# kiva12138/MIMRL

Measured on AMD Instinct MI355X. Metric: two-stage train iters/sec, higher is better.
Workload: dtype bf16

## Files before the change

mimrl_amd/csrc/cube_fused.h:

```cpp
#pragma once
#include "common.h"
#include "model_ops.h"

namespace mimrl {

struct CubeFusedArgs {
  const float* x;
  const float *l_w1, *l_b1, *l_w2, *l_b2, *l_wr, *l_g, *l_be;
  KMixW kw;
  const float *d_w1, *d_b1, *d_w2, *d_b2, *d_wr, *d_g, *d_be;
  float *l_u, *l_h, *l_y, *l_z, *l_mean, *l_rstd;
  float* k_z;
  float *d_u, *d_h, *d_y, *d_mean, *d_rstd;
  float* d_z;
  int B, il, hl, ol, K, act, save;
  int dbg_phase;
};

bool cube_fused_supported(int il, int hl, int ol, int ik, int hk, int ok, int id, int hd, int od, bool ln_first,
                          bool res_project, bool bias, const float* dropout_mlp);
int cube_block_fwd_fused(hipStream_t s, const CubeFusedArgs& a);

#ifdef MIMRL_PHASE_PROBE
int cube_fwd_read_phases(long long* out);
#endif

}
```

mimrl_amd/csrc/cube_fused.hip:

```cpp
#include "cube_fused.h"

#include "kmix_device.h"

#include <type_traits>

namespace mimrl {

namespace {

constexpr int D = 128;
constexpr int ILD = 72;
constexpr int IMG = 64 * ILD;
constexpr int CTL = 68, CTD = 132;

typedef _Float16 bf;

#ifdef MIMRL_PHASE_PROBE
__device__ long long g_cube_phase[128];
#define CPHASE(i) do { if (blockIdx.x == 0 && threadIdx.x == 0) g_cube_phase[(SAVE ? 64 : 0) + (NMT - 1) * 16 + (i)] = (long long)wall_clock64(); } while (0)
#else
#define CPHASE(i) do { } while (0)
#endif

__device__ __forceinline__ void mma64(f32x16& acc, const bf* A, const bf* B, int wm, int wn, int lane) {
#pragma unroll
  for (int s = 0; s < 4; ++s) {
    const f16x8 a = *reinterpret_cast<const f16x8*>(A + (wm * 32 + (lane & 31)) * ILD + s * 16 + 8 * (lane >> 5));
    const f16x8 b = *reinterpret_cast<const f16x8*>(B + (wn * 32 + (lane & 31)) * ILD + s * 16 + 8 * (lane >> 5));
    acc = __builtin_amdgcn_mfma_f32_32x32x16_f16(a, b, acc, 0, 0, 0);
  }
}
__device__ __forceinline__ int acc_row(int r, int wm, int lane) { return wm * 32 + (r & 3) + 8 * (r >> 2) + 4 * (lane >> 5); }

struct WReq { float v[16]; };
// ... 60 lines not shown
  c.prm = c.ksw + 256 * 4;
  const int l_end = c.prm + 4 * 64 * 4;
  c.bw = 0;
  c.dprm = c.bw + 2 * G * IMG * 2;
  int after = c.dprm + 2 * D * 4;
  if (after < xm_bytes) after = xm_bytes;
  c.az = (after + 15) & ~15;
  c.ah = c.az + nmt * 2 * IMG * 2;
  const int ah_bytes = nmt * 2 * IMG * 2, ctd_bytes = 64 * CTD * 4;
  c.ctd = c.ah;
  const int d_end = c.ah + (ah_bytes > ctd_bytes ? ah_bytes : ctd_bytes);
  c.total = l_end > d_end ? l_end : d_end;
  return c;
}

template <bool SAVE, int NMT, int G>
__global__ __launch_bounds__(256 * G) void cube_fwd_fused_kernel(CubeFusedArgs a) {
  extern __shared__ __attribute__((aligned(16))) char smem[];
  constexpr int NT = 256 * G;
  const int tid = threadIdx.x, grp = tid >> 8, t = tid & 255, lane = t & 63, wave = t >> 6, wm = wave >> 1, wn = wave & 1;
  const int b = blockIdx.x;
  const int K = a.K, C = K * D, XP = C + 8, il = a.il, hl = a.hl, ol = a.ol;
  const Carve cv = carve(K, NMT, G);
  bf* Xm = reinterpret_cast<bf*>(smem + cv.xm);
  bf* Aw = reinterpret_cast<bf*>(smem + cv.aw);
  bf* Bx = reinterpret_cast<bf*>(smem + cv.bx) + grp * IMG;
  bf* Bh = reinterpret_cast<bf*>(smem + cv.bh) + grp * IMG;
  float* CtL = reinterpret_cast<float*>(smem + cv.ctl) + grp * 64 * CTL;
  float* red = reinterpret_cast<float*>(smem + cv.red) + grp * 2 * 4 * 64;
  float* ksw = reinterpret_cast<float*>(smem + cv.ksw);
  float* prm = reinterpret_cast<float*>(smem + cv.prm);

  CPHASE(0);
  {
    const bool g0 = G == 1 || grp == 0;
    const WReq w0 = stage_weight_request(g0 ? a.l_w1 : a.l_w2, g0 ? il : hl, 0, 0, g0 ? hl : ol, g0 ? il : hl, t);
    const WReq w1 = stage_weight_request(a.l_wr, il, 0, 0, ol, il, t);
    WReq w2;
    if (G == 1) w2 = stage_weight_request(a.l_w2, hl, 0, 0, ol, hl, t);
    float pr[4] = {0.f, 0.f, 0.f, 0.f};
    if (tid < 64) {
      pr[0] = (tid < hl && a.l_b1) ? a.l_b1[tid] : 0.f;
      pr[1] = (tid < ol && a.l_b2) ? a.l_b2[tid] : 0.f;
      pr[2] = tid < ol ? a.l_g[tid] : 0.f;
      pr[3] = tid < ol ? a.l_be[tid] : 0.f;
    }
    CPHASE(13);
    const float* xb = a.x + (long)b * il * C;
    const int nq = C / 4, total = 64 * nq;
    constexpr int NQ = SAVE ? 6 : 12;
    for (int i0 = tid; i0 < total; i0 += NT * NQ) {
      float4 q[NQ];
#pragma unroll
      for (int j = 0; j < NQ; ++j) {
        const int i = i0 + NT * j;
        const int ic = i < total ? i : total - 1;
        const int l = ic / nq, c4 = (ic - l * nq) * 4;
        q[j] = *reinterpret_cast<const float4*>(xb + (long)(l < il ? l : il - 1) * C + c4);
      }
#pragma unroll
      for (int j = 0; j < NQ; ++j) {
        const int i = i0 + NT * j;
        if (!(i < total && i / nq < il)) q[j] = make_float4(0.f, 0.f, 0.f, 0.f);
      }
#pragma unroll
      for (int j = 0; j < NQ; ++j) {
        const int i = i0 + NT * j;
        if (i < total) {
          const int l = i / nq, c4 = (i - l * nq) * 4;
          f16x4 p; p[0] = to_f16_sat(q[j].x); p[1] = to_f16_sat(q[j].y); p[2] = to_f16_sat(q[j].z); p[3] = to_f16_sat(q[j].w);
          *reinterpret_cast<f16x4*>(Xm + l * XP + c4) = p;
        }
      }
    }
    CPHASE(14);
    if (tid < 64) { prm[0 * 64 + tid] = pr[0]; prm[1 * 64 + tid] = pr[1]; prm[2 * 64 + tid] = pr[2]; prm[3 * 64 + tid] = pr[3]; }
    stage_weight_commit(g0 ? Aw + 0 * IMG : Aw + 1 * IMG, w0, 0, 0, g0 ? hl : ol, g0 ? il : hl, t);
    if (g0) stage_weight_commit(Aw + 2 * IMG, w1, 0, 0, ol, il, t);
    if (G == 1) stage_weight_commit(Aw + 1 * IMG, w2, 0, 0, ol, hl, t);
  }
  __syncthreads();
  CPHASE(1);
  if (a.dbg_phase == 1) return;

  for (int nb = 0; nb < C; nb += 64 * G) {
    const int n0 = nb + 64 * grp;
    const bool on = n0 < C;
    if (on) {
// ... 123 lines not shown
        }
      }
      });
    };
    if (K == 3) phase_k(std::integral_constant<int, 3>{});
    else if (K == 1) phase_k(std::integral_constant<int, 1>{});
    else if (K == 2) phase_k(std::integral_constant<int, 2>{});
    else phase_k(std::integral_constant<int, 4>{});
  }
  __syncthreads();

  CPHASE(3);
  if (a.dbg_phase == 3) return;
  const int R = ol * K;
  float* CtD = reinterpret_cast<float*>(smem + cv.ctd);
  float* dgam = reinterpret_cast<float*>(smem + cv.dprm);
  float* dbet = dgam + D;
  bf* Az = reinterpret_cast<bf*>(smem + cv.az);
  bf* Ah = reinterpret_cast<bf*>(smem + cv.ah);
  for (int c = tid; c < NMT * 64 * 16; c += NT) {
    const int r = c >> 4, ch = c & 15;
    f16x8 v;
#pragma unroll
    for (int j = 0; j < 8; ++j) v[j] = to_f16(0.f);
    if (r < R) {
      const int l = r / K, kk = r - l * K;
      v = *reinterpret_cast<const f16x8*>(Xm + l * XP + kk * D + ch * 8);
    }
    *reinterpret_cast<f16x8*>(Az + ((r >> 6) * 2 + (ch >> 3)) * IMG + (r & 63) * ILD + (ch & 7) * 8) = v;
  }
  __syncthreads();
// ... 61 lines not shown
  CPHASE(5);
  if (a.dbg_phase == 4) return;
#pragma unroll
  for (int i = NI1; i < 3 * NI1; ++i) {
    const int which = i >= 2 * NI1, q = (i % NI1) >> 1, kh = i & 1;
    commit_weight128(Bw2[i & 1], wnext, t);
    if (i + 1 < 3 * NI1) wnext = wload(i + 1);
    __syncthreads();
    const bf* Asrc = which == 0 ? Ah : Az;
#pragma unroll
    for (int mt = 0; mt < NMT; ++mt) mma64(acc[mt][q], Asrc + (mt * 2 + kh) * IMG, Bw2[i & 1], wm, wn, lane);
  }
  __syncthreads();
  CPHASE(6);
  if (a.dbg_phase == 5) return;
#pragma unroll
  for (int mt = 0; mt < NMT; ++mt) {
#pragma unroll
    for (int q = 0; q < NTW; ++q) {
      const int n = wn * 32 + (lane & 31), col = (nt0 + q) * 64 + n;
      const float b2 = b2v[q];
#pragma unroll
      for (int r = 0; r < 16; ++r) CtD[acc_row(r, wm, lane) * CTD + col] = acc[mt][q][r] + b2;
    }
    __syncthreads();
    {
      constexpr int TPR = 4 * G, CW = 32 / G;
      const int m = tid / TPR, part = tid % TPR, row = mt * 64 + m;
      float yv[CW];
      float s0 = 0.f;
// ... 8 lines not shown
      float v0 = 0.f;
#pragma unroll
      for (int j = 0; j < CW; ++j) { const float c = yv[j] - mu; v0 += c * c; }
      v0 = group_sum<TPR>(v0);
      const float rs = rsqrtf(v0 * (1.f / D) + LN_EPS);
      if (row < R) {
        const long o = ((long)b * R + row) * D + part * CW;
#pragma unroll
        for (int j = 0; j < CW / 4; ++j) {
          const int c = part * CW + 4 * j;
          float4 z;
          z.x = (yv[4 * j] - mu) * rs * dgam[c] + dbet[c];
          z.y = (yv[4 * j + 1] - mu) * rs * dgam[c + 1] + dbet[c + 1];
          z.z = (yv[4 * j + 2] - mu) * rs * dgam[c + 2] + dbet[c + 2];
          z.w = (yv[4 * j + 3] - mu) * rs * dgam[c + 3] + dbet[c + 3];
          *reinterpret_cast<float4*>(a.d_z + o + 4 * j) = z;
          if (SAVE) *reinterpret_cast<float4*>(a.d_y + o + 4 * j) = make_float4(yv[4 * j], yv[4 * j + 1], yv[4 * j + 2], yv[4 * j + 3]);
        }
        if (SAVE && part == 0) { a.d_mean[(long)b * R + row] = mu; a.d_rstd[(long)b * R + row] = rs; }
      }
    }
    __syncthreads();
  }
  CPHASE(7);
}

}

#ifdef MIMRL_PHASE_PROBE
int cube_fwd_read_phases(long long* out) { return hipMemcpyFromSymbol(out, HIP_SYMBOL(g_cube_phase), sizeof(long long) * 128) == hipSuccess ? 0 : 1; }
#endif

bool cube_fused_supported(int il, int hl, int ol, int ik, int hk, int ok, int id, int hd, int od, bool ln_first,
                          bool res_project, bool bias, const float* dropout_mlp) {
  (void)bias;
  if (ln_first || !res_project) return false;
  if (dropout_mlp[0] > 0.f || dropout_mlp[1] > 0.f || dropout_mlp[2] > 0.f) return false;
  if (id != D || hd != D || od != D) return false;
  if (il > 64 || hl > 64 || ol > 64 || il < 1 || hl < 1 || ol < 1) return false;
  if (ik != hk || ik != ok || ik < 1 || ik > 4) return false;
  if (ol * ok > 192) return false;
  return true;
}

int cube_block_fwd_fused(hipStream_t s, const CubeFusedArgs& a) {
// ... 10 lines not shown
    HIPX(hipFuncSetAttribute(reinterpret_cast<const void*>(kern), hipFuncAttributeMaxDynamicSharedMemorySize, cv.total)); \
    hipLaunchKernelGGL(kern, dim3(a.B), dim3(256 * GG), cv.total, s, a);                                           \
  } while (0)
#define LAUNCH_NMT(SAVE, GG)                                                                                       \
  do {                                                                                                             \
    if (nmt == 1) LAUNCH_FUSED(SAVE, 1, GG); else if (nmt == 2) LAUNCH_FUSED(SAVE, 2, GG); else LAUNCH_FUSED(SAVE, 3, GG); \
  } while (0)
  if (a.save) { if (G == 1) LAUNCH_NMT(true, 1); else LAUNCH_NMT(true, 2); }
  else { if (G == 1) LAUNCH_NMT(false, 1); else LAUNCH_NMT(false, 2); }
#undef LAUNCH_NMT
#undef LAUNCH_FUSED
  LAUNCH_CHECK();
  return MIMRL_OK;
}

}
```

mimrl_amd/csrc/engine.h:

```cpp
#pragma once
#include <cstdio>
#include <cstdlib>
#include <cstring>
#include <algorithm>
#include <vector>
#include <dlfcn.h>

#include "cube_fused.h"
#include "mlp_fused.h"
#include "concat_fused.h"
#include "cube_bwd_fused.h"
#include "cube_long.h"
#include "estimator_ops.h"
#include "gemm.h"
#include "gru.h"
#include "gru_wgrad.h"
#include "concat_dw.h"
#include "lstm.h"
#include "layout.h"
#include "comm.h"
#include "model_ops.h"

namespace mimrl {

// ... 198 lines not shown
  float *dfeat = nullptr, *dtout = nullptr, *dta[3], *dtin = nullptr, *dca[3], *dP = nullptr, *dQ = nullptr;
  float *dcc[3], *dcin = nullptr;
  static constexpr int NGBUF = 24;
  float* gbuf[NGBUF];
  size_t gbuf_floats = 0;
  float *dtx = nullptr, *ds[2], *dg[2][2][2], *hprev[2][2][2], *dh0[2];

  static constexpr int NSIDE = 6;
  hipStream_t side[NSIDE] = {nullptr, nullptr, nullptr, nullptr, nullptr, nullptr};
  std::vector<hipEvent_t> ev_pool;
  size_t ev_next = 0;
  bool multi_stream = true;
  bool fused_cube_bwd = true;
  bool fused_mlp = true;
  bool fused_cube = true;
  int fwd_f16 = 1;
  int next_event(hipEvent_t* e) {
    if (ev_next == ev_pool.size()) {
      hipEvent_t n;
      HIPX(hipEventCreateWithFlags(&n, hipEventDisableTiming));
      ev_pool.push_back(n);
    }
    *e = ev_pool[ev_next++];
    return MIMRL_OK;
  }
  int G_group(hipStream_t st, const GemmDesc* ds, int n) {
    if (!prof_on) return gemm_group(st, ds, n, bf16);
    for (int i = 0; i < n; ++i) MX(G_on(st, ds[i]));
    return MIMRL_OK;
  }
// ... 143 lines not shown
  int G_(const GemmDesc& d) { return G_on(stream, d); }
  static constexpr bool fp32_site(int) { return false; }
  struct PrecGuard {
    mimrl_handle* h; bool saved;
    PrecGuard(mimrl_handle* h_, bool force_fp32) : h(h_), saved(h_->bf16) { if (force_fp32) h->bf16 = false; }
    ~PrecGuard() { h->bf16 = saved; }
  };
  struct Deferred { int kind; int side; GemmDesc g; const float* src; long n0, n1, n2, n3; float* dst;
                    const float *p1 = nullptr, *p2 = nullptr, *p3 = nullptr; float* dst2 = nullptr; KMixW kw = KMixW();
                    const float *p4 = nullptr, *p5 = nullptr; float *dst3 = nullptr, *dst4 = nullptr; };
  std::vector<Deferred> deferred;
  int flush_deferred(int only_side = 0);
  int wg_helper = -1;
  int dbg_delay(hipStream_t st, int tag);
  int model_forward(bool train, bool save, int knn_stage = 0, int part = 0);
  int cube_forward(bool train, bool save);
  int cube_backward(int cur_in, int* cur_out);
  int wt_images(hipStream_t st, bool bwd_bf16, bool launch, bool* d_fused);
  int model_backward();
  int encoders_backward(float* dcube);
  int gru_layer_backward(int l);
  struct StreamGuard {
    mimrl_handle* h; hipStream_t saved;
    StreamGuard(mimrl_handle* h_, hipStream_t st) : h(h_), saved(h_->stream) { h->stream = st; }
    ~StreamGuard() { h->stream = saved; }
  };
  int knn_launch(int stage, hipStream_t st);
  bool pipe_primed = false; int fwd_parity = 0, pipe_set = 0;
  int pipe_forward_body(bool other_inputs);
  int run_stage1_pipe_prime();
  int run_stage1_pipe(bool next_valid);
// ... 26 lines not shown
```

mimrl_amd/csrc/engine_abi.hip:

```cpp
#include "engine.h"

extern "C" {

const char* mimrl_last_error(void) { return mimrl::last_error_slot().c_str(); }
#ifdef MIMRL_PHASE_PROBE
int mimrl_dbg_cube_phases(long long* out) { return mimrl::cube_fwd_read_phases(out); }
int mimrl_dbg_cube_bwd_phases(long long* out) { return mimrl::cube_bwd_read_phases(out); }
int mimrl_dbg_kmix_phases(long long* out) { return mimrl::kmix_bwd_read_phases(out); }
int mimrl_dbg_nce_phases(long long* out) { return mimrl::nce_read_phases(out); }
int mimrl_dbg_model_ops_phases(long long* out) { return mimrl::model_ops_read_phases(out); }
int mimrl_dbg_gru_bwd_phases(long long* out) { return mimrl::gru_bwd_read_phases(out); }
int mimrl_dbg_concat_bwd_phases(long long* out) { return mimrl::concat_bwd_read_phases(out); }
#endif
int mimrl_abi_version(void) { return MIMRL_ABI_VERSION; }

int mimrl_device_check(void) {
  int n = 0;
  if (hipGetDeviceCount(&n) != hipSuccess || n <= 0) return set_error(MIMRL_ERR_NODEVICE, "no HIP device visible");
  int dev = 0;
  if (hipGetDevice(&dev) != hipSuccess) return set_error(MIMRL_ERR_NODEVICE, "hipGetDevice failed");
  hipDeviceProp_t p;
  if (hipGetDeviceProperties(&p, dev) != hipSuccess) return set_error(MIMRL_ERR_NODEVICE, "hipGetDeviceProperties failed");
  if (std::strncmp(p.gcnArchName, "gfx950", 6) != 0)
    return set_error(MIMRL_ERR_NODEVICE, "device %d is %s; this library is built for gfx950 (MI355X) only", dev, p.gcnArchName);
// ... 18 lines not shown
  MX(mimrl_device_check());
  if (knob_on("MIMRL_KNOBS")) knobs_print(stderr);
  mimrl_handle* h = new (std::nothrow) mimrl_handle();
  if (!h) return set_error(MIMRL_ERR_STATE, "out of host memory");
  h->cfg = *cfg;
  if (h->cfg.beta1 == 0.f) h->cfg.beta1 = 0.9f;
  if (h->cfg.beta2 == 0.f) h->cfg.beta2 = 0.999f;
  if (h->cfg.adam_eps == 0.f) h->cfg.adam_eps = 1e-8f;
  h->stream = h->user_stream = reinterpret_cast<hipStream_t>(hip_stream);
  h->multi_stream = knob("MIMRL_SINGLE_STREAM") == nullptr;
#ifdef MIMRL_DET
  h->multi_stream = false;
  MX(det_init());
#endif
  h->fused_cube = knob("MIMRL_NO_FUSED_CUBE") == nullptr;
  h->fused_mlp = knob("MIMRL_NO_FUSED_MLP") == nullptr;
  h->knn_pre = true;
  h->fold_unpack_on = knob("MIMRL_NO_FOLD_UNPACK") == nullptr;
  h->h16_on = knob("MIMRL_NO_H16") == nullptr;
  h->xin_on = knob("MIMRL_NO_XIN") == nullptr;
  h->fused_cube_bwd = knob("MIMRL_NO_FUSED_CUBE_BWD") == nullptr;
  h->laxis_bwd_long_on = !(knob("MIMRL_LAXIS_BWD_LONG") && atoi(knob("MIMRL_LAXIS_BWD_LONG")) == 0);
  h->laxis_long_on = !(knob("MIMRL_LAXIS_LONG") && atoi(knob("MIMRL_LAXIS_LONG")) == 0);
  h->rec16_on = !(knob("MIMRL_REC16") && atoi(knob("MIMRL_REC16")) == 0);
  h->dwih_h16_on = !(knob("MIMRL_DWIH_H16") && atoi(knob("MIMRL_DWIH_H16")) == 0);
  h->adam_frag_on = !(knob("MIMRL_ADAM_FRAG") && atoi(knob("MIMRL_ADAM_FRAG")) == 0);
  h->fused_concat = knob("MIMRL_NO_FUSED_CONCAT") == nullptr;
  h->fwd_f16 = knob("MIMRL_FWD_BF16") == nullptr;
  h->l0_packed = knob("MIMRL_L0_PACK") ? atoi(knob("MIMRL_L0_PACK")) != 0 : true;
  h->dg_bf16 = cfg->encoder == MIMRL_ENCODER_GRU && (cfg->precision & MIMRL_PREC_BF16_GRU_BWD) && (cfg->precision & MIMRL_PREC_BF16_GEMM_BWD) &&
// ... 687 lines not shown
```

mimrl_amd/csrc/engine_forward.hip:

```cpp
#include "engine.h"

int mimrl_handle::encoders_forward(bool save, int knn_stage) {
  if (cfg.encoder == MIMRL_ENCODER_CONV) return conv_forward(knn_stage);
  if (cfg.encoder == MIMRL_ENCODER_LSTM) return lstm_encoders_forward(save, knn_stage);
  const int B = cfg.batch, T = cfg.seq_len;
  const long BT_ = (long)B * T;
  const float* xin[2] = {bufs.audio, bufs.video};
  const int dmod[2] = {cfg.d_a, cfg.d_v};
  if (!ev_lens) MX(seq_lengths2(S(4), xin[0], dmod[0], lens[0], xin[1], dmod[1], lens[1], B, T));
  const bool use_h16 = h16_on && l0_packed && bf16 && fwd_f16 && (prec & MIMRL_PREC_BF16_GRU_FWD) && !fp32_site(4) && !fp32_site(2) && h0h[0] && w1h;
  if (save) { h16_live = use_h16; hp16_live = false; }
  for (int l = 0; l < 2; ++l) {
    GruFwdArgs a;
    a.B = B; a.T = T; a.out_ld = 2 * H; a.nmod = 2;
    a.btv = gru_pick_btv(B, 2);
    a.gx_f16 = gx_f16 ? 1 : 0;
    a.stamp = kstamp; a.stamp.id = l;
    if (l == 1) MX(fork(1, 3));
    if (l == 0 && !l0_packed && l0_bwd_pack && save) {
      L0Pack pk;
      for (int m = 0; m < 2; ++m) { pk.x[m] = xin[m]; pk.d[m] = dmod[m]; for (int d = 0; d < 2; ++d) { pk.w_ih[m][d] = nullptr; pk.b_ih[m][d] = nullptr; } }
      pk.xpack = xpack; pk.wpack = wpack; pk.bpack = bpack; pk.rows = BT_; pk.KP = KP();
      MX(l0_pack(S(0), pk, true, false));
    }
// ... 157 lines not shown
      g.M = rows; g.N = H; g.K = d; g.batch = B;
      if (tap == 1) g.bias_n = P(conv_b[m]); else g.beta = 1.f;
      MX(G_on(st, g));
    }
  }
  MX(join(2, 2));
  return MIMRL_OK;
}

int mimrl_handle::model_forward(bool train, bool save, int knn_stage, int part) {
  Range rg(part == 1 ? "mimrl.model_forward.prefix (Model.py:395-458)" : part == 2 ? "mimrl.model_forward.tail (Model.py:461-515)" : "mimrl.model_forward (Model.py:388-519)");
  const int B = cfg.batch, T = cfg.seq_len, L = cfg.time_len, D = cfg.d_common;
  const long BT_ = (long)B * T;
  const float pdrop[3] = {train ? cfg.dropout[0] : 0.f, train ? cfg.dropout[1] : 0.f, train ? cfg.dropout[2] : 0.f};
  if (part != 1 && T < L && !pre_done) HIPX(hipMemsetAsync(cube0, 0, sizeof(float) * (size_t)B * L * 3 * D, stream));
  static const bool fused_pre_on = knob("MIMRL_NO_FUSED_TAIL_PRE") == nullptr;
  const bool fused_pre = fused_pre_on && T <= 128;
  if (part != 2) {
    MX(fork(0, 5));
    if (cfg.encoder == MIMRL_ENCODER_GRU && side_on(0)) {
      MX(seq_lengths2(S(0), bufs.audio, cfg.d_a, lens[0], bufs.video, cfg.d_v, lens[1], B, T));
      MX(next_event(&ev_lens));
      HIPX(hipEventRecord(ev_lens, S(0)));
    }
    { PrecGuard pg(this, fp32_site(1)); GemmDesc g = gemm_nt(bufs.text, cfg.d_t, P(w_t), cfg.d_t, tx_raw, D, (int)BT_, D, cfg.d_t); g.f16 = fwd_f16; MX(G_on(S(0), g)); }
    MX(dbg_delay(S(0), 10));
    if (part == 0 && !fused_pre) MX(text_post_fwd(S(0), tx_raw, cube0, B, T, L, 3, D, 0, pdrop[0], key(), 0));
    MX(encoders_forward(save, knn_stage));
    MX(join(0, 0));
    if (part == 1) return MIMRL_OK;
  } else if (!fused_pre && !pre_done) {
    MX(text_post_fwd(stream, tx_raw, cube0, B, T, L, 3, D, 0, pdrop[0], key(), 0));
  }
  if (!pre_done) {
    LnSide2 sd[2];
    for (int m = 0; m < 2; ++m)
      sd[m] = LnSide2{h1[m], P(ln_g[m]), P(ln_b[m]), ln_mean[m], ln_rstd[m], nullptr, nullptr, nullptr, 1 + m, pdrop[1 + m],
                      (uint32_t)(1 + m)};
    if (fused_pre) {
      MX(tail_pre_fwd(stream, tx_raw, pdrop[0], sd[0], sd[1], cube0, bufs.feats + (size_t)B * D, B, T, L, 3, D, key()));
    } else {
      MX(ln_relu_drop_fwd2(stream, sd[0], sd[1], cube0, B, T, L, 3, D, key()));
      MX(feat_mean_fwd(stream, cube0, bufs.feats + (size_t)B * D, B, T, L, 3, D));
    }
  }
  { Scope sc(this, MIMRL_PH_CUBE_FWD); MX(cube_forward(train, save)); }
  MX(dbg_delay(stream, save ? 2 : 13));
  const BlockBuf& last = bb[cfg.n_blocks - 1];
  const int ol = cfg.d_outs[cfg.n_blocks - 1][0], ok = cfg.d_outs[cfg.n_blocks - 1][1], od = cfg.d_outs[cfg.n_blocks - 1][2];
  if (od != D) return set_error(MIMRL_ERR_ARG, "last block d_out must equal d_common (features feed 128-wide estimators)");
  MX(head_fwd(stream, last.d.z, P(cls_w), P(cls_b), bufs.feats, bufs.pred, B, ol, ok, od, cfg.compose_t_sum,
              cfg.compose_k_sum));
  (void)ff;
  return MIMRL_OK;
}

int mimrl_handle::dual_tail_pre() {
  const int B = cfg.batch, T = cfg.seq_len, L = cfg.time_len, D = cfg.d_common;
  float* const cubes[2] = {cube0, alt.cube0};
  float* const feats[2] = {bufs.feats + (size_t)B * D, alt.feats + (size_t)B * D};
  const int add[2] = {1, 0};
  if (T < L)
    for (int o = 0; o < 2; ++o) HIPX(hipMemsetAsync(cubes[o], 0, sizeof(float) * (size_t)B * L * 3 * D, stream));
  LnSide2 sd[2];
  for (int m = 0; m < 2; ++m)
    sd[m] = LnSide2{h1[m], P(ln_g[m]), P(ln_b[m]), ln_mean[m], ln_rstd[m], nullptr, nullptr, nullptr, 1 + m, cfg.dropout[1 + m], (uint32_t)(1 + m)};
  MX(tail_pre2_fwd(stream, tx_raw, cfg.dropout[0], sd[0], sd[1], cubes, feats, add, tailp_part, B, T, L, 3, D, key()));
  return MIMRL_OK;
}

int mimrl_handle::cube_forward(bool train, bool save) {
  const int B = cfg.batch;
  const float* x = cube0;
  int il = cfg.time_len, ik = 3, id = cfg.d_common;
  const bool no_fused = !fused_cube;
  for (int i = 0; i < cfg.n_blocks; ++i) {
    const BlockW& w = blk[i];
    BlockBuf& b = bb[i];
    const int hl = w.ax[0].hid, ol = w.ax[0].out, hk = w.ax[1].hid, ok = w.ax[1].out, hd = w.ax[2].hid, od = w.ax[2].out;
    const float pl = train ? cfg.dropout_mlp[0] : 0.f, pk = train ? cfg.dropout_mlp[1] : 0.f,
                pd = train ? cfg.dropout_mlp[2] : 0.f;
    const float pmlp[3] = {pl, pk, pd};
    if (bf16 && !no_fused &&
        cube_fused_supported(il, hl, ol, ik, hk, ok, id, hd, od, cfg.ln_first != 0, cfg.res_project[i] != 0, cfg.bias != 0, pmlp)) {
      CubeFusedArgs fa;
      std::memset(&fa, 0, sizeof fa);
      auto PB = [&](long off) -> const float* { return off >= 0 ? P(off) : nullptr; };
      fa.x = x;
      fa.l_w1 = P(w.ax[0].fc1.w); fa.l_b1 = PB(w.ax[0].fc1.b); fa.l_w2 = P(w.ax[0].fc2.w); fa.l_b2 = PB(w.ax[0].fc2.b);
      fa.l_wr = P(w.ax[0].res); fa.l_g = P(w.ax[0].ln_g); fa.l_be = P(w.ax[0].ln_b);
      fa.kw.w1 = P(w.ax[1].fc1.w); fa.kw.b1 = PB(w.ax[1].fc1.b); fa.kw.w2 = P(w.ax[1].fc2.w); fa.kw.b2 = PB(w.ax[1].fc2.b);
      fa.kw.wr = P(w.ax[1].res); fa.kw.g = P(w.ax[1].ln_g); fa.kw.be = P(w.ax[1].ln_b);
      fa.kw.ik = ik; fa.kw.hk = hk; fa.kw.ok = ok; fa.kw.act = cfg.activation; fa.kw.ln_first = 0; fa.kw.drop_p = 0.f;
      fa.kw.key = key(); fa.kw.stream_id = 0;
      fa.d_w1 = P(w.ax[2].fc1.w); fa.d_b1 = PB(w.ax[2].fc1.b); fa.d_w2 = P(w.ax[2].fc2.w); fa.d_b2 = PB(w.ax[2].fc2.b);
      fa.d_wr = P(w.ax[2].res); fa.d_g = P(w.ax[2].ln_g); fa.d_be = P(w.ax[2].ln_b);
      if (save) {
        fa.l_u = b.l.u; fa.l_h = b.l.h; fa.l_y = b.l.y; fa.l_z = b.l.z; fa.l_mean = b.l.mean; fa.l_rstd = b.l.rstd;
        fa.k_z = b.k.z;
        fa.d_u = b.d.u; fa.d_h = b.d.h; fa.d_y = b.d.y; fa.d_mean = b.d.mean; fa.d_rstd = b.d.rstd;
      }
      fa.d_z = b.d.z;
      fa.dbg_phase = dbg_env("MIMRL_CUBE_PHASE") ? atoi(dbg_env("MIMRL_CUBE_PHASE")) : 0;
      fa.B = B; fa.il = il; fa.hl = hl; fa.ol = ol; fa.K = ik; fa.act = cfg.activation; fa.save = save ? 1 : 0;
      if (fa.dbg_phase == 100) { fa.save = 0; fa.dbg_phase = 0; }
      MX(cube_block_fwd_fused(stream, fa));
      x = b.d.z;
      il = ol; ik = ok; id = od;
      continue;
    }
    {
      const AxisW& a = w.ax[0];
      const long C = (long)ik * id;
      const float* xi = x;
      const bool long_l = bf16 && laxis_long_on && !cfg.ln_first && pl <= 0.f && a.res >= 0 && laxis_fwd_long_supported(il, hl, ol, (int)C);
      if (long_l) {
        if (w2p[i] && hl % 4 != 0) {
          MX(pad_rows(stream, P(a.fc2.w), w2p[i], ol, hl, (hl + 3) & ~3));
          w2p_valid[i] = true;
        }
// ... 108 lines not shown
```

mimrl_amd/csrc/knobs.cpp:

```cpp
#include "knobs.h"

#include <cstdlib>
#include <cstring>
#include <mutex>
#include <set>
#include <string>

namespace mimrl {

namespace {
struct KnobDef { const char* name; const char* where; const char* dflt; const char* help; };
const KnobDef kKnobs[] = {
  {"MIMRL_KNOBS", "engine_abi.hip", "", "1: print this table (values in effect) to stderr when a handle is created"},
  {"MIMRL_ADAM_FRAG", "engine_abi.hip", "", "0: combined step with frag_images + stage_boundary as launches behind the critic Adam (round 5a) instead of inside it"},
  {"MIMRL_CONCAT_STREAMED", "concat_fused.hip", "", "1: the concat critic on the weight-streaming kernels of rounds 2-5 (concat_fused.hip) instead of the weights-stationary ones (concat_ws.hip)"},
  {"MIMRL_DBG_DELAY_TAG", "engine_backward.hip", "-1", "critical-path probe: <tag>[:<us>] -- the phase tag behind which a spin kernel of <us> (default 50) microseconds is injected (tools/critical_path.sh)"},
  {"MIMRL_DDP_SPLIT", "engine_abi.hip", "", "0: the main gradient bucket all-reduced in one piece (in-library RCCL and dist.py)"},
  {"MIMRL_DG_FP32", "engine_abi.hip", "", "BPTT outputs dg / h_prev stored as fp32 instead of bf16"},
  {"MIMRL_DWIH_H16", "engine_abi.hip", "", "0: the layer-1 dW_ih product reads the fp32 layer-0 outputs instead of the recurrence's fp16 copy"},
  {"MIMRL_FWD_BF16", "engine_abi.hip", "", "forward products round to bf16 instead of fp16"},
  {"MIMRL_GEMM_TALL_MIN_M", "gemm_tall.hip", "", "row threshold of the tall LDS-DMA GEMM (default 4096)"},
  {"MIMRL_GRAPH_DOT", "engine_step.hip", "", "dump the captured two-stage graph to this file (hipGraphDebugDotPrint)"},
  {"MIMRL_GRU_LDS_PAD", "gru.hip", "-1", "KiB of dynamic LDS a small BPTT launch reserves to keep parked kernels off its CUs (default 144 below 129 workgroups)"},
  {"MIMRL_GRU_SKIP", "gru.hip", "0", "probe build only (make probe): phase-elimination mask of the recurrence kernels; ignored by the default build"},
// ... 4 lines not shown
  {"MIMRL_NO_GRU_WGRAD", "engine_backward.hip", "", "1: the layer-0 GRU weight gradients as two batched split-K GEMMs instead of the one-pass kernel (gru_wgrad.hip, round 6)"},
  {"MIMRL_LAXIS_BWD_LONG", "engine_abi.hip", "", "0: the L-axis backward of a long-sequence CubeMLP block (L > 64) as colln_bwd + GEMM chain instead of the LONG instantiation of laxis_bwd_kernel"},
  {"MIMRL_LAXIS_LONG", "engine_abi.hip", "", "0: the L-axis MLP of a long-sequence CubeMLP block (L > 64) as the GEMM chain instead of the one-pass kernel of cube_long.hip"},
  {"MIMRL_LSTM_MFMA_FP32", "lstm.hip", "", "1: fp32 precision mode runs the fp32-MFMA LSTM kernels instead of the scalar ones (measured slower)"},
  {"MIMRL_LSTM_SCALAR", "lstm.hip", "", "1: the scalar fp32 LSTM kernels of round 1 instead of the MFMA ones"},
  {"MIMRL_MLP_NO_FRAG", "mlp_fused.hip", "", "the round-2 kernels (read per call: tests/test_gpu_fused_oracle.py toggles it)"},
  {"MIMRL_NO_FOLD_UNPACK", "engine_abi.hip", "", "packed layer-0 weight gradients through l0_unpack instead of the Adam fold"},
  {"MIMRL_NO_FUSED_CONCAT", "engine_abi.hip", "", "concat critic tail as a GEMM chain instead of concat_fwd / concat_bwd"},
  {"MIMRL_NO_FUSED_CUBE", "engine_abi.hip", "", "bf16 mode: CubeMLP forward as the unfused GEMM / LayerNorm chain"},
  {"MIMRL_NO_FUSED_CUBE_BWD", "engine_abi.hip", "", "bf16 mode: CubeMLP backward as the unfused chain"},
  {"MIMRL_NO_FUSED_MI", "engine_estimators.hip", "", "separable critic: scores / bound / gradients as separate kernels instead of mi_sep_fused / mi_sep_nce"},
  {"MIMRL_NO_FUSED_MLP", "engine_abi.hip", "", "bf16 mode: estimator MLP stacks as grouped GEMMs"},
  {"MIMRL_NO_FUSED_MLP_BWD", "engine_estimators.hip", "", "estimator MLP stacks: data-gradient chain as GEMMs instead of the fused kernel"},
  {"MIMRL_NO_CONCAT_DQ", "engine_estimators.hip", "", "concat critic backward: dZ0 goes out in fp32 and pair_reduce_q sums it over the x rows (rounds 2-4) instead of the in-kernel dQ partial sums"},
  {"MIMRL_NO_DUAL_TAIL_PRE", "engine_step.hip", "", "long sequences (T > 128): each forward tail runs its own text dropout / LN + ReLU + dropout / temporal-mean launches instead of one launch for both"},
  {"MIMRL_NO_FUSED_TAIL_PRE", "engine_forward.hip", "", "forward tail: text dropout, LN + ReLU + dropout and the temporal means as separate launches"},
  {"MIMRL_NO_GEMM_TALL", "gemm_tall.hip", "", "tall LDS-DMA GEMM (gemm_tall.hip) off: the 128x128 register-staged kernels"},
  {"MIMRL_NO_H16", "engine_abi.hip", "", "fp32-stored operands for the layer-1 projection / dh0 (bit-identical results)"},
  {"MIMRL_NO_MI_NCE_TILED", "engine_estimators.hip", "", "separable InfoNCE: the one-workgroup-per-estimator kernel instead of the row-tiled one"},
  {"MIMRL_NO_SHARED_PREFIX", "engine_step.hip", "", "evaluate the prefix twice"},
  {"MIMRL_NO_STEP_GRAPH", "engine_step.hip", "", "Solver.step as two per-stage graphs instead of one combined graph"},
  {"MIMRL_NO_XIN", "engine_abi.hip", "", "layer-0 input projection as its own GEMM instead of fused into the recurrence kernel"},
  {"MIMRL_REC16", "engine_abi.hip", "", "0: the BPTT launches read fp32 dout / h_prev (round 5a): dh0 and ds stored fp32, the fused-projection forward writes its fp32 outputs"},
  {"MIMRL_SINGLE_STREAM", "engine_abi.hip", "", "enqueue everything on one stream (no side streams)"},
};
constexpr int kN = sizeof(kKnobs) / sizeof(kKnobs[0]);
}

const char* knob(const char* name) {
  bool known = false;
  for (int i = 0; i < kN && !known; ++i) known = std::strcmp(kKnobs[i].name, name) == 0;
// ... 25 lines not shown
```

Baseline: 1270.

## Chain both CubeMLP blocks and the classifier head into one forward kernel

Adds cube_tail_fused_kernel, which runs the first CubeMLP block, keeps its output in LDS as fp16, runs the second block on it and then computes the temporal/modal mean and linear head in the same workgroup. It applies only to the non-saving forward with two blocks. This removes two kernel launches and the global round trip of the intermediate d_z and the last block's output. Next-block weights are prefetched during the first block's epilogue. In exchange, LDS use grows to the larger block's carve plus extra space. The MIMRL_NO_FUSED_TAIL_PRE knob is also removed, so the fused tail-pre path is now always used when T <= 128.

Result: faster. 1286 (median of 6 runs) (+1.2%).

```diff
diff --git a/mimrl_amd/csrc/cube_fused.h b/mimrl_amd/csrc/cube_fused.h
--- a/mimrl_amd/csrc/cube_fused.h
+++ b/mimrl_amd/csrc/cube_fused.h
@@ -21,6 +21,10 @@
                           bool res_project, bool bias, const float* dropout_mlp);
 int cube_block_fwd_fused(hipStream_t s, const CubeFusedArgs& a);
 
+struct CubeTailHead { const float *w, *bias; float *feats, *pred; int sum_l, sum_k; };
+bool cube_tail_fused_supported(int n_blocks, bool blk0_fused, bool blk1_fused, const CubeFusedArgs& a0, const CubeFusedArgs& a1, int od_last);
+int cube_tail_fwd_fused(hipStream_t s, const CubeFusedArgs& a0, const CubeFusedArgs& a1, const CubeTailHead& h);
+
 #ifdef MIMRL_PHASE_PROBE
 int cube_fwd_read_phases(long long* out);
 #endif
diff --git a/mimrl_amd/csrc/cube_fused.hip b/mimrl_amd/csrc/cube_fused.hip
--- a/mimrl_amd/csrc/cube_fused.hip
+++ b/mimrl_amd/csrc/cube_fused.hip
@@ -16,8 +16,8 @@
 typedef _Float16 bf;
 
 #ifdef MIMRL_PHASE_PROBE
-__device__ long long g_cube_phase[128];
-#define CPHASE(i) do { if (blockIdx.x == 0 && threadIdx.x == 0) g_cube_phase[(SAVE ? 64 : 0) + (NMT - 1) * 16 + (i)] = (long long)wall_clock64(); } while (0)
+__device__ long long g_cube_phase[256];
+#define CPHASE(i) do { if (blockIdx.x == 0 && threadIdx.x == 0) g_cube_phase[PBASE + (i)] = (long long)wall_clock64(); } while (0)
 #else
 #define CPHASE(i) do { } while (0)
 #endif
@@ -108,10 +108,30 @@
   return c;
 }
 
-template <bool SAVE, int NMT, int G>
-__global__ __launch_bounds__(256 * G) void cube_fwd_fused_kernel(CubeFusedArgs a) {
-  extern __shared__ __attribute__((aligned(16))) char smem[];
+enum { TAIL_IN_XM = 1, TAIL_OUT_XM = 2, TAIL_HEAD = 4 };
+struct LReq { WReq w0, w1; float pr[4]; };
+struct TailHead { const float *w, *bias; float *ff, *pred; float scale; };
+
+template <int G>
+__device__ __forceinline__ void l_request(const CubeFusedArgs& a, int tid, int grp, int t, LReq& r) {
+  const int il = a.il, hl = a.hl, ol = a.ol;
+  const bool g0 = G == 1 || grp == 0;
+  r.w0 = stage_weight_request(g0 ? a.l_w1 : a.l_w2, g0 ? il : hl, 0, 0, g0 ? hl : ol, g0 ? il : hl, t);
+  r.w1 = stage_weight_request(a.l_wr, il, 0, 0, ol, il, t);
+  r.pr[0] = r.pr[1] = r.pr[2] = r.pr[3] = 0.f;
+  if (tid < 64) {
+    r.pr[0] = (tid < hl && a.l_b1) ? a.l_b1[tid] : 0.f;
+    r.pr[1] = (tid < ol && a.l_b2) ? a.l_b2[tid] : 0.f;
+    r.pr[2] = tid < ol ? a.l_g[tid] : 0.f;
+    r.pr[3] = tid < ol ? a.l_be[tid] : 0.f;
+  }
+}
+
+template <bool SAVE, int NMT, int G, int MODE, int PBASE>
+__device__ __forceinline__ void cube_block(const CubeFusedArgs& a, const CubeFusedArgs& na, const TailHead& hd, LReq& lr, char* smem, int dprm_off) {
   constexpr int NT = 256 * G;
+  constexpr bool IN_XM = (MODE & TAIL_IN_XM) != 0, OUT_XM = (MODE & TAIL_OUT_XM) != 0, HEAD = (MODE & TAIL_HEAD) != 0;
+  static_assert(MODE == 0 || G == 2, "the chained forms are built for two wave groups");
   const int tid = threadIdx.x, grp = tid >> 8, t = tid & 255, lane = t & 63, wave = t >> 6, wm = wave >> 1, wn = wave & 1;
   const int b = blockIdx.x;
   const int K = a.K, C = K * D, XP = C + 8, il = a.il, hl = a.hl, ol = a.ol;
@@ -128,18 +148,13 @@
   CPHASE(0);
   {
     const bool g0 = G == 1 || grp == 0;
-    const WReq w0 = stage_weight_request(g0 ? a.l_w1 : a.l_w2, g0 ? il : hl, 0, 0, g0 ? hl : ol, g0 ? il : hl, t);
-    const WReq w1 = stage_weight_request(a.l_wr, il, 0, 0, ol, il, t);
+    if constexpr (!IN_XM) l_request<G>(a, tid, grp, t, lr);
     WReq w2;
     if (G == 1) w2 = stage_weight_request(a.l_w2, hl, 0, 0, ol, hl, t);
-    float pr[4] = {0.f, 0.f, 0.f, 0.f};
-    if (tid < 64) {
-      pr[0] = (tid < hl && a.l_b1) ? a.l_b1[tid] : 0.f;
-      pr[1] = (tid < ol && a.l_b2) ? a.l_b2[tid] : 0.f;
-      pr[2] = tid < ol ? a.l_g[tid] : 0.f;
-      pr[3] = tid < ol ? a.l_be[tid] : 0.f;
-    }
+    const WReq &w0 = lr.w0, &w1 = lr.w1;
+    const float* pr = lr.pr;
     CPHASE(13);
+    if constexpr (!IN_XM) {
     const float* xb = a.x + (long)b * il * C;
     const int nq = C / 4, total = 64 * nq;
     constexpr int NQ = SAVE ? 6 : 12;
@@ -166,6 +181,7 @@
           *reinterpret_cast<f16x4*>(Xm + l * XP + c4) = p;
         }
       }
+    }
     }
     CPHASE(14);
     if (tid < 64) { prm[0 * 64 + tid] = pr[0]; prm[1 * 64 + tid] = pr[1]; prm[2 * 64 + tid] = pr[2]; prm[3 * 64 + tid] = pr[3]; }
@@ -319,7 +335,7 @@
   if (a.dbg_phase == 3) return;
   const int R = ol * K;
   float* CtD = reinterpret_cast<float*>(smem + cv.ctd);
-  float* dgam = reinterpret_cast<float*>(smem + cv.dprm);
+  float* dgam = reinterpret_cast<float*>(smem + (dprm_off >= 0 ? dprm_off : cv.dprm));
   float* dbet = dgam + D;
   bf* Az = reinterpret_cast<bf*>(smem + cv.az);
   bf* Ah = reinterpret_cast<bf*>(smem + cv.ah);
@@ -411,6 +427,20 @@
   __syncthreads();
   CPHASE(6);
   if (a.dbg_phase == 5) return;
+  float* Ht = reinterpret_cast<float*>(smem);
+  float hw = 0.f, hbias = 0.f;
+  if constexpr (OUT_XM) {
+    if constexpr (!SAVE) l_request<G>(na, tid, grp, t, lr);
+    const int cpr = C / 8;
+    f16x8 z8;
+#pragma unroll
+    for (int j = 0; j < 8; ++j) z8[j] = to_f16(0.f);
+    for (int i = tid; i < (64 - ol) * cpr; i += NT) {
+      const int l = ol + i / cpr, c8 = (i - (i / cpr) * cpr) * 8;
+      *reinterpret_cast<f16x8*>(Xm + l * XP + c8) = z8;
+    }
+  }
+  if constexpr (HEAD) { hw = hd.w[tid & 127]; hbias = hd.bias[0]; }
 #pragma unroll
   for (int mt = 0; mt < NMT; ++mt) {
 #pragma unroll
@@ -449,7 +479,13 @@
           z.y = (yv[4 * j + 1] - mu) * rs * dgam[c + 1] + dbet[c + 1];
           z.z = (yv[4 * j + 2] - mu) * rs * dgam[c + 2] + dbet[c + 2];
           z.w = (yv[4 * j + 3] - mu) * rs * dgam[c + 3] + dbet[c + 3];
-          *reinterpret_cast<float4*>(a.d_z + o + 4 * j) = z;
+          if constexpr (!OUT_XM || SAVE) *reinterpret_cast<float4*>(a.d_z + o + 4 * j) = z;
+          if constexpr (OUT_XM) {
+            const int l = row / K, kk = row - l * K;
+            f16x4 p; p[0] = to_f16_sat(z.x); p[1] = to_f16_sat(z.y); p[2] = to_f16_sat(z.z); p[3] = to_f16_sat(z.w);
+            *reinterpret_cast<f16x4*>(Xm + l * XP + kk * D + c) = p;
+          }
+          if constexpr (HEAD) *reinterpret_cast<float4*>(Ht + row * D + c) = z;
           if (SAVE) *reinterpret_cast<float4*>(a.d_y + o + 4 * j) = make_float4(yv[4 * j], yv[4 * j + 1], yv[4 * j + 2], yv[4 * j + 3]);
         }
         if (SAVE && part == 0) { a.d_mean[(long)b * R + row] = mu; a.d_rstd[(long)b * R + row] = rs; }
@@ -458,12 +494,54 @@
     __syncthreads();
   }
   CPHASE(7);
+  if constexpr (OUT_XM && SAVE) l_request<G>(na, tid, grp, t, lr);
+  if constexpr (HEAD) {
+    static_assert(NT == 512, "the head's reduction is head_fwd_kernel's 512-thread one");
+    float* ph = CtD;
+    float* hred = CtD + 4 * D;
+    const int d = tid & 127, q = tid >> 7;
+    float s = 0.f;
+#pragma unroll 8
+    for (int i = q; i < R; i += 4) s += Ht[i * D + d];
+    ph[q * D + d] = s;
+    __syncthreads();
+    float part = 0.f;
+    if (q == 0) {
+      s = ((ph[d] + ph[D + d]) + (ph[2 * D + d] + ph[3 * D + d])) * hd.scale;
+      hd.ff[(long)b * D + d] = s;
+      part = s * hw;
+    }
+    part = block_sum(part, hred);
+    if (tid == 0) hd.pred[b] = part + hbias;
+    CPHASE(15);
+  }
+}
+
+template <bool SAVE, int NMT, int G>
+__global__ __launch_bounds__(256 * G) void cube_fwd_fused_kernel(CubeFusedArgs a) {
+  extern __shared__ __attribute__((aligned(16))) char smem[];
+  LReq lr;
+  cube_block<SAVE, NMT, G, 0, (SAVE ? 64 : 0) + (NMT - 1) * 16>(a, a, TailHead{}, lr, smem, -1);
+}
+
+struct TailArgs { CubeFusedArgs a0, a1; TailHead hd; int dprm_off; };
+template <bool SAVE, int NMT0, int NMT1>
+__global__ __launch_bounds__(512) void cube_tail_fused_kernel(TailArgs ta) {
+  extern __shared__ __attribute__((aligned(16))) char smem[];
+  LReq lr;
+  cube_block<SAVE, NMT0, 2, TAIL_OUT_XM, 128 + (SAVE ? 64 : 0)>(ta.a0, ta.a1, ta.hd, lr, smem, ta.dprm_off);
+  typedef const __attribute__((address_space(4))) char* kptr;
+  const kptr kp = (kptr)__builtin_amdgcn_kernarg_segment_ptr();
+  unsigned off = 0;
+  asm volatile("" : "+s"(off));
+  const TailArgs& tl = *(const TailArgs*)(kp + off);
+  cube_block<SAVE, NMT1, 2, TAIL_IN_XM | TAIL_HEAD, 128 + (SAVE ? 64 : 0) + 16>(tl.a1, tl.a1, tl.hd, lr, smem, tl.dprm_off);
 }
 
 }
 
 #ifdef MIMRL_PHASE_PROBE
-int cube_fwd_read_phases(long long* out) { return hipMemcpyFromSymbol(out, HIP_SYMBOL(g_cube_phase), sizeof(long long) * 128) == hipSuccess ? 0 : 1; }
+int cube_fwd_read_phases(long long* out) { return hipMemcpyFromSymbol(out, HIP_SYMBOL(g_cube_phase), sizeof(long long) * 256) == hipSuccess ? 0 : 1; }
 #endif
 
 bool cube_fused_supported(int il, int hl, int ol, int ik, int hk, int ok, int id, int hd, int od, bool ln_first,
@@ -504,4 +582,44 @@
   return MIMRL_OK;
 }
 
-}
+static int tail_lds(const CubeFusedArgs& a0, const CubeFusedArgs& a1, int* dprm_off) {
+  const Carve c0 = carve(a0.K, (a0.ol * a0.K + 63) / 64, 2), c1 = carve(a1.K, (a1.ol * a1.K + 63) / 64, 2);
+  const int body = ((c0.total > c1.total ? c0.total : c1.total) + 15) & ~15;
+  if (dprm_off) *dprm_off = body;
+  return body + 2 * D * 4;
+}
+
+bool cube_tail_fused_supported(int n_blocks, bool blk0_fused, bool blk1_fused, const CubeFusedArgs& a0, const CubeFusedArgs& a1, int od_last) {
+  if (n_blocks != 2 || !blk0_fused || !blk1_fused) return false;
+  if (a1.il != a0.ol || a0.K != a1.K || od_last != D) return false;
+  if (a0.save != a1.save || a0.act != a1.act || a0.dbg_phase != 0 || a1.dbg_phase != 0) return false;
+  const int n0 = (a0.ol * a0.K + 63) / 64, n1 = (a1.ol * a1.K + 63) / 64;
+  if (n0 < 1 || n0 > 3 || n1 < 1 || n1 > 3) return false;
+  if (a0.save) return false;
+  return tail_lds(a0, a1, nullptr) <= 160 * 1024;
+}
+
+int cube_tail_fwd_fused(hipStream_t s, const CubeFusedArgs& a0, const CubeFusedArgs& a1, const CubeTailHead& h) {
+  const int n0 = (a0.ol * a0.K + 63) / 64, n1 = (a1.ol * a1.K + 63) / 64;
+  int dprm_off = 0;
+  const int lds = tail_lds(a0, a1, &dprm_off);
+  if (lds > 160 * 1024 || a0.save || a1.save || n0 > 3 || n1 > 3) return set_error(MIMRL_ERR_ARG, "cube_tail_fused: unsupported configuration");
+  const TailArgs ta{a0, a1, TailHead{h.w, h.bias, h.feats, h.pred, (h.sum_l ? 1.f : 1.f / a1.ol) * (h.sum_k ? 1.f : 1.f / a1.K)}, dprm_off};
+#define LAUNCH_TAIL(N0, N1)                                                                                        \
+  do {                                                                                                             \
+    auto kern = cube_tail_fused_kernel<false, N0, N1>;                                                             \
+    HIPX(hipFuncSetAttribute(reinterpret_cast<const void*>(kern), hipFuncAttributeMaxDynamicSharedMemorySize, lds)); \
+    hipLaunchKernelGGL(kern, dim3(a0.B), dim3(512), lds, s, ta);                                                   \
+  } while (0)
+#define LAUNCH_TAIL_N1(N0)                                                                                         \
+  do {                                                                                                             \
+    if (n1 == 1) LAUNCH_TAIL(N0, 1); else if (n1 == 2) LAUNCH_TAIL(N0, 2); else LAUNCH_TAIL(N0, 3);                \
+  } while (0)
+  if (n0 == 1) LAUNCH_TAIL_N1(1); else if (n0 == 2) LAUNCH_TAIL_N1(2); else LAUNCH_TAIL_N1(3);
+#undef LAUNCH_TAIL_N1
+#undef LAUNCH_TAIL
+  LAUNCH_CHECK();
+  return MIMRL_OK;
+}
+
+}
diff --git a/mimrl_amd/csrc/engine.h b/mimrl_amd/csrc/engine.h
--- a/mimrl_amd/csrc/engine.h
+++ b/mimrl_amd/csrc/engine.h
@@ -236,6 +236,7 @@
   bool fused_cube_bwd = true;
   bool fused_mlp = true;
   bool fused_cube = true;
+  bool fused_tail = true;
   int fwd_f16 = 1;
   int next_event(hipEvent_t* e) {
     if (ev_next == ev_pool.size()) {
@@ -409,7 +410,8 @@
   int wg_helper = -1;
   int dbg_delay(hipStream_t st, int tag);
   int model_forward(bool train, bool save, int knn_stage = 0, int part = 0);
-  int cube_forward(bool train, bool save);
+  int cube_forward(bool train, bool save, bool* head_done = nullptr);
+  void cube_fused_args(int i, const float* x, int il, int ik, bool save, CubeFusedArgs* out);
   int cube_backward(int cur_in, int* cur_out);
   int wt_images(hipStream_t st, bool bwd_bf16, bool launch, bool* d_fused);
   int model_backward();
diff --git a/mimrl_amd/csrc/engine_abi.hip b/mimrl_amd/csrc/engine_abi.hip
--- a/mimrl_amd/csrc/engine_abi.hip
+++ b/mimrl_amd/csrc/engine_abi.hip
@@ -56,6 +56,7 @@
   MX(det_init());
 #endif
   h->fused_cube = knob("MIMRL_NO_FUSED_CUBE") == nullptr;
+  h->fused_tail = knob("MIMRL_NO_FUSED_TAIL") == nullptr;
   h->fused_mlp = knob("MIMRL_NO_FUSED_MLP") == nullptr;
   h->knn_pre = true;
   h->fold_unpack_on = knob("MIMRL_NO_FOLD_UNPACK") == nullptr;
diff --git a/mimrl_amd/csrc/engine_forward.hip b/mimrl_amd/csrc/engine_forward.hip
--- a/mimrl_amd/csrc/engine_forward.hip
+++ b/mimrl_amd/csrc/engine_forward.hip
@@ -195,8 +195,7 @@
   const long BT_ = (long)B * T;
   const float pdrop[3] = {train ? cfg.dropout[0] : 0.f, train ? cfg.dropout[1] : 0.f, train ? cfg.dropout[2] : 0.f};
   if (part != 1 && T < L && !pre_done) HIPX(hipMemsetAsync(cube0, 0, sizeof(float) * (size_t)B * L * 3 * D, stream));
-  static const bool fused_pre_on = knob("MIMRL_NO_FUSED_TAIL_PRE") == nullptr;
-  const bool fused_pre = fused_pre_on && T <= 128;
+  const bool fused_pre = T <= 128;
   if (part != 2) {
     MX(fork(0, 5));
     if (cfg.encoder == MIMRL_ENCODER_GRU && side_on(0)) {
@@ -225,13 +224,15 @@
       MX(feat_mean_fwd(stream, cube0, bufs.feats + (size_t)B * D, B, T, L, 3, D));
     }
   }
-  { Scope sc(this, MIMRL_PH_CUBE_FWD); MX(cube_forward(train, save)); }
-  MX(dbg_delay(stream, save ? 2 : 13));
   const BlockBuf& last = bb[cfg.n_blocks - 1];
   const int ol = cfg.d_outs[cfg.n_blocks - 1][0], ok = cfg.d_outs[cfg.n_blocks - 1][1], od = cfg.d_outs[cfg.n_blocks - 1][2];
   if (od != D) return set_error(MIMRL_ERR_ARG, "last block d_out must equal d_common (features feed 128-wide estimators)");
-  MX(head_fwd(stream, last.d.z, P(cls_w), P(cls_b), bufs.feats, bufs.pred, B, ol, ok, od, cfg.compose_t_sum,
-              cfg.compose_k_sum));
+  bool head_done = false;
+  { Scope sc(this, MIMRL_PH_CUBE_FWD); MX(cube_forward(train, save, &head_done)); }
+  MX(dbg_delay(stream, save ? 2 : 13));
+  if (!head_done)
+    MX(head_fwd(stream, last.d.z, P(cls_w), P(cls_b), bufs.feats, bufs.pred, B, ol, ok, od, cfg.compose_t_sum,
+                cfg.compose_k_sum));
   (void)ff;
   return MIMRL_OK;
 }
@@ -250,41 +251,66 @@
   return MIMRL_OK;
 }
 
-int mimrl_handle::cube_forward(bool train, bool save) {
+void mimrl_handle::cube_fused_args(int i, const float* x, int il, int ik, bool save, CubeFusedArgs* out) {
+  const BlockW& w = blk[i];
+  BlockBuf& b = bb[i];
+  const int hl = w.ax[0].hid, ol = w.ax[0].out, hk = w.ax[1].hid, ok = w.ax[1].out;
+  CubeFusedArgs& fa = *out;
+  std::memset(&fa, 0, sizeof fa);
+  auto PB = [&](long off) -> const float* { return off >= 0 ? P(off) : nullptr; };
+  fa.x = x;
+  fa.l_w1 = P(w.ax[0].fc1.w); fa.l_b1 = PB(w.ax[0].fc1.b); fa.l_w2 = P(w.ax[0].fc2.w); fa.l_b2 = PB(w.ax[0].fc2.b);
+  fa.l_wr = P(w.ax[0].res); fa.l_g = P(w.ax[0].ln_g); fa.l_be = P(w.ax[0].ln_b);
+  fa.kw.w1 = P(w.ax[1].fc1.w); fa.kw.b1 = PB(w.ax[1].fc1.b); fa.kw.w2 = P(w.ax[1].fc2.w); fa.kw.b2 = PB(w.ax[1].fc2.b);
+  fa.kw.wr = P(w.ax[1].res); fa.kw.g = P(w.ax[1].ln_g); fa.kw.be = P(w.ax[1].ln_b);
+  fa.kw.ik = ik; fa.kw.hk = hk; fa.kw.ok = ok; fa.kw.act = cfg.activation; fa.kw.ln_first = 0; fa.kw.drop_p = 0.f;
+  fa.kw.key = key(); fa.kw.stream_id = 0;
+  fa.d_w1 = P(w.ax[2].fc1.w); fa.d_b1 = PB(w.ax[2].fc1.b); fa.d_w2 = P(w.ax[2].fc2.w); fa.d_b2 = PB(w.ax[2].fc2.b);
+  fa.d_wr = P(w.ax[2].res); fa.d_g = P(w.ax[2].ln_g); fa.d_be = P(w.ax[2].ln_b);
+  if (save) {
+    fa.l_u = b.l.u; fa.l_h = b.l.h; fa.l_y = b.l.y; fa.l_z = b.l.z; fa.l_mean = b.l.mean; fa.l_rstd = b.l.rstd;
+    fa.k_z = b.k.z;
+    fa.d_u = b.d.u; fa.d_h = b.d.h; fa.d_y = b.d.y; fa.d_mean = b.d.mean; fa.d_rstd = b.d.rstd;
+  }
+  fa.d_z = b.d.z;
+  fa.dbg_phase = dbg_env("MIMRL_CUBE_PHASE") ? atoi(dbg_env("MIMRL_CUBE_PHASE")) : 0;
+  fa.B = cfg.batch; fa.il = il; fa.hl = hl; fa.ol = ol; fa.K = ik; fa.act = cfg.activation; fa.save = save ? 1 : 0;
+  if (fa.dbg_phase == 100) { fa.save = 0; fa.dbg_phase = 0; }
+}
+
+int mimrl_handle::cube_forward(bool train, bool save, bool* head_done) {
   const int B = cfg.batch;
   const float* x = cube0;
   int il = cfg.time_len, ik = 3, id = cfg.d_common;
   const bool no_fused = !fused_cube;
+  const float pl = train ? cfg.dropout_mlp[0] : 0.f, pk = train ? cfg.dropout_mlp[1] : 0.f,
+              pd = train ? cfg.dropout_mlp[2] : 0.f;
+  const float pmlp[3] = {pl, pk, pd};
+  auto blk_fused = [&](int i, int il_, int ik_, int id_) {
+    const BlockW& w = blk[i];
+    return bf16 && !no_fused &&
+           cube_fused_supported(il_, w.ax[0].hid, w.ax[0].out, ik_, w.ax[1].hid, w.ax[1].out, id_, w.ax[2].hid, w.ax[2].out, cfg.ln_first != 0,
+                                cfg.res_project[i] != 0, cfg.bias != 0, pmlp);
+  };
+  if (head_done && fused_tail && cfg.n_blocks == 2 && blk_fused(0, il, ik, id) &&
+      blk_fused(1, blk[0].ax[0].out, blk[0].ax[1].out, blk[0].ax[2].out)) {
+    CubeFusedArgs a0, a1;
+    cube_fused_args(0, x, il, ik, save, &a0);
+    cube_fused_args(1, bb[0].d.z, blk[0].ax[0].out, blk[0].ax[1].out, save, &a1);
+    if (cube_tail_fused_supported(cfg.n_blocks, true, true, a0, a1, blk[1].ax[2].out)) {
+      const CubeTailHead th{P(cls_w), P(cls_b), bufs.feats, bufs.pred, cfg.compose_t_sum, cfg.compose_k_sum};
+      MX(cube_tail_fwd_fused(stream, a0, a1, th));
+      *head_done = true;
+      return MIMRL_OK;
+    }
+  }
   for (int i = 0; i < cfg.n_blocks; ++i) {
     const BlockW& w = blk[i];
     BlockBuf& b = bb[i];
     const int hl = w.ax[0].hid, ol = w.ax[0].out, hk = w.ax[1].hid, ok = w.ax[1].out, hd = w.ax[2].hid, od = w.ax[2].out;
-    const float pl = train ? cfg.dropout_mlp[0] : 0.f, pk = train ? cfg.dropout_mlp[1] : 0.f,
-                pd = train ? cfg.dropout_mlp[2] : 0.f;
-    const float pmlp[3] = {pl, pk, pd};
-    if (bf16 && !no_fused &&
-        cube_fused_supported(il, hl, ol, ik, hk, ok, id, hd, od, cfg.ln_first != 0, cfg.res_project[i] != 0, cfg.bias != 0, pmlp)) {
+    if (blk_fused(i, il, ik, id)) {
       CubeFusedArgs fa;
-      std::memset(&fa, 0, sizeof fa);
-      auto PB = [&](long off) -> const float* { return off >= 0 ? P(off) : nullptr; };
-      fa.x = x;
-      fa.l_w1 = P(w.ax[0].fc1.w); fa.l_b1 = PB(w.ax[0].fc1.b); fa.l_w2 = P(w.ax[0].fc2.w); fa.l_b2 = PB(w.ax[0].fc2.b);
-      fa.l_wr = P(w.ax[0].res); fa.l_g = P(w.ax[0].ln_g); fa.l_be = P(w.ax[0].ln_b);
-      fa.kw.w1 = P(w.ax[1].fc1.w); fa.kw.b1 = PB(w.ax[1].fc1.b); fa.kw.w2 = P(w.ax[1].fc2.w); fa.kw.b2 = PB(w.ax[1].fc2.b);
-      fa.kw.wr = P(w.ax[1].res); fa.kw.g = P(w.ax[1].ln_g); fa.kw.be = P(w.ax[1].ln_b);
-      fa.kw.ik = ik; fa.kw.hk = hk; fa.kw.ok = ok; fa.kw.act = cfg.activation; fa.kw.ln_first = 0; fa.kw.drop_p = 0.f;
-      fa.kw.key = key(); fa.kw.stream_id = 0;
-      fa.d_w1 = P(w.ax[2].fc1.w); fa.d_b1 = PB(w.ax[2].fc1.b); fa.d_w2 = P(w.ax[2].fc2.w); fa.d_b2 = PB(w.ax[2].fc2.b);
-      fa.d_wr = P(w.ax[2].res); fa.d_g = P(w.ax[2].ln_g); fa.d_be = P(w.ax[2].ln_b);
-      if (save) {
-        fa.l_u = b.l.u; fa.l_h = b.l.h; fa.l_y = b.l.y; fa.l_z = b.l.z; fa.l_mean = b.l.mean; fa.l_rstd = b.l.rstd;
-        fa.k_z = b.k.z;
-        fa.d_u = b.d.u; fa.d_h = b.d.h; fa.d_y = b.d.y; fa.d_mean = b.d.mean; fa.d_rstd = b.d.rstd;
-      }
-      fa.d_z = b.d.z;
-      fa.dbg_phase = dbg_env("MIMRL_CUBE_PHASE") ? atoi(dbg_env("MIMRL_CUBE_PHASE")) : 0;
-      fa.B = B; fa.il = il; fa.hl = hl; fa.ol = ol; fa.K = ik; fa.act = cfg.activation; fa.save = save ? 1 : 0;
-      if (fa.dbg_phase == 100) { fa.save = 0; fa.dbg_phase = 0; }
+      cube_fused_args(i, x, il, ik, save, &fa);
       MX(cube_block_fwd_fused(stream, fa));
       x = b.d.z;
       il = ol; ik = ok; id = od;
diff --git a/mimrl_amd/csrc/knobs.cpp b/mimrl_amd/csrc/knobs.cpp
--- a/mimrl_amd/csrc/knobs.cpp
+++ b/mimrl_amd/csrc/knobs.cpp
@@ -42,7 +42,7 @@
   {"MIMRL_NO_FUSED_MLP_BWD", "engine_estimators.hip", "", "estimator MLP stacks: data-gradient chain as GEMMs instead of the fused kernel"},
   {"MIMRL_NO_CONCAT_DQ", "engine_estimators.hip", "", "concat critic backward: dZ0 goes out in fp32 and pair_reduce_q sums it over the x rows (rounds 2-4) instead of the in-kernel dQ partial sums"},
   {"MIMRL_NO_DUAL_TAIL_PRE", "engine_step.hip", "", "long sequences (T > 128): each forward tail runs its own text dropout / LN + ReLU + dropout / temporal-mean launches instead of one launch for both"},
-  {"MIMRL_NO_FUSED_TAIL_PRE", "engine_forward.hip", "", "forward tail: text dropout, LN + ReLU + dropout and the temporal means as separate launches"},
+  {"MIMRL_NO_FUSED_TAIL", "engine_abi.hip", "", "bf16 mode: the non-saving forward tail as two block launches + head_fwd instead of the chained cube_tail_fused_kernel"},
   {"MIMRL_NO_GEMM_TALL", "gemm_tall.hip", "", "tall LDS-DMA GEMM (gemm_tall.hip) off: the 128x128 register-staged kernels"},
   {"MIMRL_NO_H16", "engine_abi.hip", "", "fp32-stored operands for the layer-1 projection / dh0 (bit-identical results)"},
   {"MIMRL_NO_MI_NCE_TILED", "engine_estimators.hip", "", "separable InfoNCE: the one-workgroup-per-estimator kernel instead of the row-tiled one"},
```
